# reidprichard/ORC

Hardware: AMD Instinct MI355X
Metric: SIMPLE iterations/s (10.24M-cell hex channel equivalents; = iterations/s at N=1) (higher is better)
Workload: dtype f64

## Files before the change

orc_amd/csrc/linalg_kernels.hpp:

```cpp
#pragma once
#include "linalg.hpp"

namespace orc {

__device__ __forceinline__ double view_value(const MatView &A, int64_t row, int64_t pos) {
    double v = A.val[pos];
    if (A.s1) v = A.s1[row] * v;
    if (A.s2) v = A.s2[row] * v;
    return v;
}

template <bool NT, class T>
__device__ __forceinline__ T ld_stream(const T *p) {
    if (NT) return __builtin_nontemporal_load(p);
    return *p;
}

typedef unsigned u32x4_t __attribute__((ext_vector_type(4)));
typedef int i32x2_t __attribute__((ext_vector_type(2)));
typedef double f64x2_t __attribute__((ext_vector_type(2)));
typedef unsigned u32x3_t __attribute__((ext_vector_type(3)));
typedef u32x3_t u32x3_a4_t __attribute__((aligned(4)));
template <bool NT>
__device__ __forceinline__ u32x3_t ld_pos12(const unsigned *p) {
    if (NT) return __builtin_nontemporal_load(reinterpret_cast<const u32x3_a4_t *>(p));
    return *reinterpret_cast<const u32x3_a4_t *>(p);
}

__device__ __forceinline__ int packed_pair(bool in, int &off) {
    const unsigned long long m = __ballot(in);
    const int rank = __builtin_amdgcn_mbcnt_hi((unsigned)(m >> 32), __builtin_amdgcn_mbcnt_lo((unsigned)m, 0u));
    const int p = in ? off + rank : (m != 0ull ? off : off - 1);
    off += __popcll(m);
    return p;
}

__device__ __forceinline__ double fold_partials_block(const double *__restrict__ partials, int count, double *lds16 ) {
    const int lane = threadIdx.x & 63, w = threadIdx.x >> 6;
    double a[4], b[4];
#pragma unroll
    for (int p = 0; p < 4; ++p) {
        const int vt = (w + 4 * p) * 64 + lane;
        a[p] = vt < count ? partials[vt] : 0.;
        b[p] = vt + 1024 < count ? partials[vt + 1024] : 0.;
    }
    __syncthreads();
#pragma unroll
    for (int p = 0; p < 4; ++p) {
        const int vt = (w + 4 * p) * 64 + lane;
        double v = 0.;
        if (vt < count) v += a[p];
        if (vt + 1024 < count) v += b[p];
        v = wave_sum(v);
        if (lane == 0) lds16[w + 4 * p] = v;
    }
    __syncthreads();
    double r = 0.;
#pragma unroll
    for (int i = 0; i < 16; ++i) r += lds16[i];
    return r;
}

template <int NQ>
__device__ __forceinline__ void fold_partials_multi(const double *__restrict__ partials, int count, double *lds , double (&out)[NQ]) {
    const int lane = threadIdx.x & 63, w = threadIdx.x >> 6;
    double a[NQ][4], b[NQ][4];
#pragma unroll
    for (int q = 0; q < NQ; ++q) {
#pragma unroll
        for (int p = 0; p < 4; ++p) {
            const int vt = (w + 4 * p) * 64 + lane;
            a[q][p] = vt < count ? partials[(size_t)q * count + vt] : 0.;
            b[q][p] = vt + 1024 < count ? partials[(size_t)q * count + vt + 1024] : 0.;
        }
    }
    __syncthreads();
#pragma unroll
    for (int q = 0; q < NQ; ++q) {
#pragma unroll
        for (int p = 0; p < 4; ++p) {
            const int vt = (w + 4 * p) * 64 + lane;
            double v = 0.;
            if (vt < count) v += a[q][p];
            if (vt + 1024 < count) v += b[q][p];
            v = wave_sum(v);
            if (lane == 0) lds[q * 16 + w + 4 * p] = v;
        }
    }
    __syncthreads();
#pragma unroll
    for (int q = 0; q < NQ; ++q) {
        double r = 0.;
#pragma unroll
        for (int i = 0; i < 16; ++i) r += lds[q * 16 + i];
        out[q] = r;
    }
}

struct SliceWalk {
    int64_t begin, end, step;
    __device__ __forceinline__ SliceWalk(int32_t n_slices, int32_t first = 0) : SliceWalk(n_slices, first, (int)blockIdx.x, (int)gridDim.x) {}
    __device__ __forceinline__ SliceWalk(int32_t n_slices, int32_t first, int block, int grid) {
        const int waves = blockDim.x >> 6;
        const int wave = __builtin_amdgcn_readfirstlane((int)(threadIdx.x >> 6));
        if ((grid & 7) == 0 && grid >= 8) {
            const int xcd = block & 7, bl = block >> 3, nb = grid >> 3;
            const int64_t spx = ((int64_t)(n_slices - first) + 7) / 8;
            const int64_t lo = (int64_t)first + (int64_t)xcd * spx;
            int64_t hi = lo + spx;
            if (hi > n_slices) hi = n_slices;
            begin = lo + (int64_t)bl * waves + wave;
            end = hi;
            step = (int64_t)nb * waves;
        } else {
            begin = (int64_t)first + (int64_t)block * waves + wave;
            end = n_slices;
            step = (int64_t)grid * waves;
        }
    }
};

enum { kSpmvPlain = 0, kSpmvRagged = 1, kSpmvPacked = 2 };
template <class Epi, int kLayout = kSpmvPlain, bool kNoGather = false, bool kGuard = false>
__global__ __launch_bounds__(kBlock) void spmv_k(MatView A, const double *__restrict__ x, Epi epi, double *__restrict__ partials,
                                                 const double *__restrict__ skip_flags ) {
    __shared__ double lds[8];
    if (skip_flags && (skip_flags[0] != 0. || skip_flags[1] != 0.)) return;
    const int lane = threadIdx.x & 63;
    double r0 = 0., r1 = 0.;
    SliceWalk w(A.P.n_slices);
    for (int64_t slice = w.begin; slice < w.end; slice += w.step) {
        const int64_t row = slice * 64 + lane;
        const int64_t base = A.P.slice_ptr[slice];
        const int width = (int)((A.P.slice_ptr[slice + 1] - base) >> 6);
        const bool live = row < A.P.n;
        const int len = live ? A.P.row_len[row] : 0;
        const double s1 = (A.s1 && live) ? A.s1[row] : 1.;
        const double s2 = (A.s2 && live) ? A.s2[row] : 1.;
        double acc = 0.;
        const i32x2_t *pk_c = kLayout == kSpmvPacked ? reinterpret_cast<const i32x2_t *>(A.pk.col + A.pk.ptr[slice]) : nullptr;
        const f64x2_t *pk_v = kLayout == kSpmvPacked ? reinterpret_cast<const f64x2_t *>(A.pk.val + A.pk.ptr[slice]) : nullptr;
        int pk_off = 0;
        const int last = (kLayout == kSpmvRagged ? (len > 0 ? len : 1) : width) - 1;
        const int lane_c = live ? lane : (int)((A.P.n - 1) & 63);
        for (int k0 = 0; k0 < width; k0 += 8) {
            int c[8];
            double v[8], xv[8];
            if (kLayout == kSpmvPacked) {
#pragma unroll
                for (int q = 0; q < 4; ++q) {
                    const int p = packed_pair(k0 + 2 * q < len, pk_off);
                    const i32x2_t cc = pk_c[p];
                    const f64x2_t vv = pk_v[p];
                    c[2 * q] = cc.x; c[2 * q + 1] = cc.y;
                    v[2 * q] = vv.x; v[2 * q + 1] = vv.y;
                }
            } else {
#pragma unroll
                for (int u = 0; u < 8; ++u) {
                    if (kGuard) {
                        if (k0 + u < width) {
                            const int kk = kLayout == kSpmvPlain ? k0 + u : (k0 + u < last ? k0 + u : last);
                            const int64_t p = kLayout == kSpmvPlain ? (base + (int64_t)k0 * 64 + lane_c) + (int64_t)u * 64 : base + (int64_t)kk * 64 + lane_c;
                            c[u] = A.P.col[p];
                            v[u] = A.val[p];
                        } else { c[u] = 0; v[u] = 0.; }
                    } else {
                        const int kk = k0 + u < last ? k0 + u : last;
                        const int64_t p = base + (int64_t)kk * 64 + lane_c;
                        c[u] = A.P.col[p];
                        v[u] = A.val[p];
                    }
                }
            }
#pragma unroll
            for (int u = 0; u < 8; ++u) {
                if (kGuard) { if (k0 + u < width) xv[u] = x[c[u]]; else xv[u] = 0.; }
                else xv[u] = x[kNoGather ? (int)(live ? row : 0) + (c[u] & 0) : c[u]];
            }
#pragma unroll
            for (int u = 0; u < 8; ++u) {
                double t = v[u];
                if (A.s1) t = s1 * t;
                if (A.s2) t = s2 * t;
                const double next = acc + t * xv[u];
                acc = (k0 + u < len) ? next : acc;
            }
        }
        if (live) epi.apply(row, acc, r0, r1);
    }
    if (Epi::kReductions > 0) {
        double t = block_sum(r0, lds);
        if (threadIdx.x == 0) partials[blockIdx.x] = t;
    }
    if (Epi::kReductions > 1) {
        double t = block_sum(r1, lds);
        if (threadIdx.x == 0) partials[gridDim.x + blockIdx.x] = t;
    }
}

template <class Epi, bool kRagged = false, bool kMesh = false, bool kNarrow = false, bool kScaled = true, bool kNT = false>
__global__ __launch_bounds__(kBlock) void spmv_uniform_k(MatView A, const double *__restrict__ x, Epi epi, double *__restrict__ partials,
                                                 const double *__restrict__ skip_flags ) {
    __shared__ double lds[8];
    if (skip_flags && (skip_flags[0] != 0. || skip_flags[1] != 0.)) return;
    const int lane = threadIdx.x & 63;
    double r0 = 0., r1 = 0.;
    SliceWalk w(A.slice_hi >= 0 ? A.slice_hi : A.P.n_slices, A.slice_lo);
    for (int64_t slice = w.begin; slice < w.end; slice += w.step) {
        const int64_t row = slice * 64 + lane;
        const int64_t base = A.P.slice_ptr[slice];
        const int width = (int)((A.P.slice_ptr[slice + 1] - base) >> 6);
        const bool live = row < A.P.n;
        const int len = live ? A.P.row_len[row] : 0;
        const double s1 = (kScaled && A.s1 && live) ? A.s1[row] : 1.;
        const double s2 = (kScaled && A.s2 && live) ? A.s2[row] : 1.;
        double acc = 0.;
        const int32_t *__restrict__ cb = kNarrow ? A.P.colbase + (base >> 6) : nullptr;
        for (int k0 = 0; k0 < width; k0 += 8) {
            int c[8];
            double v[8], xv[8];
            const int64_t p0 = base + (int64_t)k0 * 64 + lane;
            if (kNarrow) {
#pragma unroll
                for (int u = 0; u < 8; ++u) {
                    const bool in = k0 + u < width;
                    c[u] = in ? cb[k0 + u] + (int)ld_stream<kNT>(A.P.col16 + p0 + (int64_t)u * 64) : 0;
                    v[u] = in ? ld_stream<kNT>(A.val + p0 + (int64_t)u * 64) : 0.;
                }
            } else {
#pragma unroll
                for (int u = 0; u < 8; ++u) {
                    const bool in = k0 + u < (kRagged ? len : width);
                    c[u] = in ? ld_stream<kNT>(A.P.col + p0 + (int64_t)u * 64) : 0;
                    v[u] = in ? ld_stream<kNT>(A.val + p0 + (int64_t)u * 64) : 0.;
                }
            }
#pragma unroll
            for (int u = 0; u < 8; ++u) xv[u] = (k0 + u < len) ? x[c[u]] : 0.;
#pragma unroll
            for (int u = 0; u < 8; ++u) {
                if (k0 + u < len) {
                    double t = v[u];
                    if (kScaled && A.s1) t = s1 * t;
                    if (kScaled && A.s2) t = s2 * t;
                    acc += t * xv[u];
                }
            }
        }
        if (live) epi.apply(row, acc, r0, r1);
    }
    const int pstride = A.part_stride > 0 ? A.part_stride : (int)gridDim.x;
    if (Epi::kReductions > 0) {
        double t = block_sum(r0, lds);
        if (threadIdx.x == 0) partials[A.part_base + blockIdx.x] = t;
    }
    if (Epi::kReductions > 1) {
        double t = block_sum(r1, lds);
        if (threadIdx.x == 0) partials[pstride + A.part_base + blockIdx.x] = t;
    }
}


struct __attribute__((aligned(8))) Vec3d { double a, b, c; };

template <class Epi3, int kChunk = 4, bool kMesh = false, bool kNarrow = false, bool kScaled = true, bool kNT = false>
__global__ __launch_bounds__(kBlock) void spmv3_uniform_k(MatView3 A, const double *__restrict__ x3, Epi3 epi, double *__restrict__ partials) {
    __shared__ double lds[8];
    const int lane = threadIdx.x & 63;
    const Vec3d *__restrict__ xv3 = reinterpret_cast<const Vec3d *>(x3);
    const Vec3d *__restrict__ s1v = reinterpret_cast<const Vec3d *>(A.s1);
    const Vec3d *__restrict__ s2v = reinterpret_cast<const Vec3d *>(A.s2);
    const int vgrid = (int)gridDim.x;
    for (int vb = blockIdx.x; vb < vgrid; vb += gridDim.x) {
    double red[3][2] = {{0., 0.}, {0., 0.}, {0., 0.}};
    SliceWalk w(A.slice_hi >= 0 ? A.slice_hi : A.P.n_slices, A.slice_lo, vb, vgrid);
    for (int64_t slice = w.begin; slice < w.end; slice += w.step) {
        const int64_t row = slice * 64 + lane;
        const int64_t base = A.P.slice_ptr[slice];
        const int width = (int)((A.P.slice_ptr[slice + 1] - base) >> 6);
        const bool live = row < A.P.n;
        const int len = live ? A.P.row_len[row] : 0;
        Vec3d s1 = {1., 1., 1.}, s2 = {1., 1., 1.};
        if (kScaled && A.s1 && live) s1 = s1v[row];
        if (kScaled && A.s2 && live) s2 = s2v[row];
        double acc0 = 0., acc1 = 0., acc2 = 0.;
        const int32_t *__restrict__ cb = kNarrow ? A.P.colbase + (base >> 6) : nullptr;
        for (int k0 = 0; k0 < width; k0 += kChunk) {
            int c[kChunk];
            double v0[kChunk], v1[kChunk], v2[kChunk];
            Vec3d xv[kChunk];
            const int64_t p0 = base + (int64_t)k0 * 64 + lane;
#pragma unroll
            for (int u = 0; u < kChunk; ++u) {
                const bool in = k0 + u < width;
                if (kNarrow) c[u] = in ? cb[k0 + u] + (int)ld_stream<kNT>(A.P.col16 + p0 + (int64_t)u * 64) : 0;
                else c[u] = in ? ld_stream<kNT>(A.P.col + p0 + (int64_t)u * 64) : 0;
                v0[u] = in ? ld_stream<kNT>(A.val[0] + p0 + (int64_t)u * 64) : 0.;
                v1[u] = in ? ld_stream<kNT>(A.val[1] + p0 + (int64_t)u * 64) : 0.;
                v2[u] = in ? ld_stream<kNT>(A.val[2] + p0 + (int64_t)u * 64) : 0.;
            }
#pragma unroll
            for (int u = 0; u < kChunk; ++u) {
                if (k0 + u < len) xv[u] = xv3[c[u]];
                else xv[u] = Vec3d{0., 0., 0.};
            }
#pragma unroll
            for (int u = 0; u < kChunk; ++u) {
                if (k0 + u < len) {
                    double t0 = v0[u], t1 = v1[u], t2 = v2[u];
                    if (kScaled && A.s1) { t0 = s1.a * t0; t1 = s1.b * t1; t2 = s1.c * t2; }
                    if (kScaled && A.s2) { t0 = s2.a * t0; t1 = s2.b * t1; t2 = s2.c * t2; }
                    acc0 += t0 * xv[u].a;
                    acc1 += t1 * xv[u].b;
                    acc2 += t2 * xv[u].c;
                }
            }
        }
        if (live) {
            const double acc[3] = {acc0, acc1, acc2};
            epi.apply(row, acc, red);
        }
    }
#pragma unroll
    for (int s = 0; s < 3; ++s) {
#pragma unroll
        for (int q = 0; q < Epi3::kReductions; ++q) {
            const double t = block_sum(red[s][q], lds);
            if (threadIdx.x == 0) partials[(size_t)(s * Epi3::kReductions + q) * (A.part_stride > 0 ? A.part_stride : vgrid) + A.part_base + vb] = t;
        }
    }
    }
}

template <class Epi, bool kScaled = true, bool kNT = false, bool kP12 = false>
__global__ __launch_bounds__(kBlock) void spmv_xwin_k(MatView A, const double *__restrict__ x, Epi epi, double *__restrict__ partials,
                                                      const double *__restrict__ skip_flags) {
    __shared__ double lds[8];
    extern __shared__ __align__(16) double xs[];
    constexpr int kC = kPackChunk;
    if (skip_flags && (skip_flags[0] != 0. || skip_flags[1] != 0.)) return;
    const int lane = threadIdx.x & 63, wave = __builtin_amdgcn_readfirstlane((int)(threadIdx.x >> 6));
    double r0 = 0., r1 = 0.;
    const int64_t n_blocks = ((int64_t)A.P.n_slices + 3) >> 2;
    int64_t b_begin, b_end, b_step;
    if ((gridDim.x & 7) == 0 && gridDim.x >= 8) {
        const int xcd = blockIdx.x & 7, bl = blockIdx.x >> 3, nb = gridDim.x >> 3;
        const int64_t per = (n_blocks + 7) / 8;
        b_begin = (int64_t)xcd * per + bl;
        b_end = (int64_t)(xcd + 1) * per < n_blocks ? (int64_t)(xcd + 1) * per : n_blocks;
        b_step = nb;
    } else {
        b_begin = blockIdx.x; b_end = n_blocks; b_step = gridDim.x;
    }
    for (int64_t b = b_begin; b < b_end; b += b_step) {
        const int ws_built = A.xw.wsize[b];
        const int ws = ws_built <= A.xw.cap ? ws_built : -1;
        const int64_t slice = b * 4 + wave;
        const bool has_slice = slice < A.P.n_slices;
        const int64_t row = slice * 64 + lane;
        const bool live = has_slice && row < A.P.n;
        int width = 0, len = 0;
        int64_t pk_off = 0, lp_off = 0;
        if (has_slice) {
            const int64_t base = A.P.slice_ptr[slice];
            width = (int)((A.P.slice_ptr[slice + 1] - base) >> 6);
            len = live ? A.P.row_len[row] : 0;
            pk_off = A.pk.ptr[slice];
            lp_off = ws >= 0 ? A.xw.lptr[slice] : 0;
        }
        const int64_t sb = __builtin_amdgcn_readfirstlane((int)(pk_off & 0xffffffff)) | ((int64_t)__builtin_amdgcn_readfirstlane((int)(pk_off >> 32)) << 32);
        const int64_t lb = __builtin_amdgcn_readfirstlane((int)(lp_off & 0xffffffff)) | ((int64_t)__builtin_amdgcn_readfirstlane((int)(lp_off >> 32)) << 32);
        const u32x4_t *s_pos = reinterpret_cast<const u32x4_t *>(A.xw.lidx + lb);
        const unsigned *s_pos12 = reinterpret_cast<const unsigned *>(A.xw.lidx) + (lb >> 3) * 3;
        const f64x2_t *s_val = reinterpret_cast<const f64x2_t *>(A.pk.val + sb);
        int poff = 0, voff = 0;
        u32x4_t c, cn;
        f64x2_t v[kC / 2], vn[kC / 2];
        auto issue = [&](int k0, u32x4_t &cc, f64x2_t (&vv)[kC / 2]) {
            {
                const unsigned long long m = __ballot(k0 < len);
                const int rank = __builtin_amdgcn_mbcnt_hi((unsigned)(m >> 32), __builtin_amdgcn_mbcnt_lo((unsigned)m, 0u));
                const int slot = poff + (k0 < len ? rank : 0);
                if (kP12) {
                    const u32x3_t w = ld_pos12<kNT>(s_pos12 + 3 * slot);
                    cc = u32x4_t{w.x, w.y, w.z, 0u};
                } else {
                    cc = ld_stream<kNT>(s_pos + slot);
                }
                poff += __popcll(m);
            }
#pragma unroll
            for (int q = 0; q < kC / 2; ++q) vv[q] = ld_stream<kNT>(s_val + packed_pair(k0 + 2 * q < len, voff));
        };
        if (ws > 0 && A.xw.wfmt[b]) {
            const int nseg = (ws + kXWinSeg - 1) / kXWinSeg;
            const int32_t *wb = A.xw.wcol + b * kXWinCap;
            const uint16_t *w16 = reinterpret_cast<const uint16_t *>(wb + nseg);
            for (int j0 = 0; j0 < ws; j0 += 8 * kBlock) {
                int wj[8];
                double xw[8];
#pragma unroll
                for (int q = 0; q < 8; ++q) {
                    const int j = j0 + q * kBlock + (int)threadIdx.x;
                    const int seg = min((j0 + q * kBlock + wave * 64) / kXWinSeg, nseg - 1);
                    wj[q] = wb[seg] + (int)ld_stream<kNT>(w16 + (j < ws ? j : ws - 1));
                }
#pragma unroll
                for (int q = 0; q < 8; ++q) xw[q] = x[wj[q]];
#pragma unroll
                for (int q = 0; q < 8; ++q) {
                    const int j = j0 + q * kBlock + (int)threadIdx.x;
                    if (j < ws) xs[j] = xw[q];
                }
            }
        } else if (ws > 0) {
            const int32_t *wc = A.xw.wcol + b * kXWinCap;
            for (int j0 = 0; j0 < ws; j0 += 8 * kBlock) {
                int wj[8];
                double xw[8];
#pragma unroll
                for (int q = 0; q < 8; ++q) {
                    const int j = j0 + q * kBlock + (int)threadIdx.x;
                    wj[q] = ld_stream<kNT>(wc + (j < ws ? j : 0));
                }
#pragma unroll
                for (int q = 0; q < 8; ++q) xw[q] = x[wj[q]];
#pragma unroll
                for (int q = 0; q < 8; ++q) {
                    const int j = j0 + q * kBlock + (int)threadIdx.x;
                    if (j < ws) xs[j] = xw[q];
                }
            }
        }
        __syncthreads();
        if (has_slice) {
            const double s1 = (kScaled && A.s1 && live) ? A.s1[row] : 1.;
            const double s2 = (kScaled && A.s2 && live) ? A.s2[row] : 1.;
            double acc = 0.;
            if (ws >= 0) {
                auto consume = [&](int k0, const u32x4_t &cc, const f64x2_t (&vv)[kC / 2]) {
                    double xv[kC];
                    if (kP12) {
                        const unsigned w0 = cc[0], w1 = cc[1], w2 = cc[2];
                        const unsigned o[kC] = {w0 << 3, w0 >> 9, __builtin_amdgcn_alignbit(w1, w0, 21), w1 >> 1, w1 >> 13, __builtin_amdgcn_alignbit(w2, w1, 25), w2 >> 5, w2 >> 17};
#pragma unroll
                        for (int u = 0; u < kC; ++u) xv[u] = *reinterpret_cast<const double *>(reinterpret_cast<const char *>(xs) + (o[u] & 0x7ff8u));
                    } else {
#pragma unroll
                        for (int q = 0; q < kC / 2; ++q) {
                            const unsigned w = cc[q];
                            xv[2 * q] = xs[w & 0xffffu];
                            xv[2 * q + 1] = xs[w >> 16];
                        }
                    }
#pragma unroll
                    for (int u = 0; u < kC; ++u) {
                        double t = vv[u >> 1][u & 1];
                        if (kScaled && A.s1) t = s1 * t;
                        if (kScaled && A.s2) t = s2 * t;
                        const double next = acc + t * xv[u];
                        acc = (k0 + u < len) ? next : acc;
                    }
                };
                if (width > 0) issue(0, c, v);
                int k0 = 0;
                for (; k0 + kC < width; k0 += 2 * kC) {
                    issue(k0 + kC, cn, vn);
                    consume(k0, c, v);
                    if (k0 + 2 * kC < width) issue(k0 + 2 * kC, c, v);
                    consume(k0 + kC, cn, vn);
                }
                if (k0 < width) consume(k0, c, v);
            } else {
                const i32x2_t *s_col = reinterpret_cast<const i32x2_t *>(A.pk.col + sb);
                for (int k0 = 0; k0 < width; k0 += 8) {
                    int cg[8];
                    double vg[8], xv[8];
#pragma unroll
                    for (int q = 0; q < 4; ++q) {
                        const int p = packed_pair(k0 + 2 * q < len, voff);
                        const i32x2_t cc = ld_stream<kNT>(s_col + p);
                        const f64x2_t vv = ld_stream<kNT>(s_val + p);
                        cg[2 * q] = cc.x; cg[2 * q + 1] = cc.y;
                        vg[2 * q] = vv.x; vg[2 * q + 1] = vv.y;
                    }
#pragma unroll
                    for (int u = 0; u < 8; ++u) xv[u] = x[cg[u]];
#pragma unroll
                    for (int u = 0; u < 8; ++u) {
                        double t = vg[u];
                        if (kScaled && A.s1) t = s1 * t;
                        if (kScaled && A.s2) t = s2 * t;
                        const double next = acc + t * xv[u];
                        acc = (k0 + u < len) ? next : acc;
                    }
                }
            }
            if (live) epi.apply(row, acc, r0, r1);
        }
        __syncthreads();
    }
    if (Epi::kReductions > 0 && A.xw.fold_scratch) {
        __shared__ int s_last;
        const int nwg = (int)gridDim.x;
        const double t0 = block_sum(r0, lds);
        const double t1 = Epi::kReductions > 1 ? block_sum(r1, lds) : 0.;
        if (threadIdx.x == 0) {
            __hip_atomic_store(A.xw.fold_scratch + blockIdx.x, t0, __ATOMIC_RELAXED, __HIP_MEMORY_SCOPE_AGENT);
            if (Epi::kReductions > 1) __hip_atomic_store(A.xw.fold_scratch + nwg + blockIdx.x, t1, __ATOMIC_RELAXED, __HIP_MEMORY_SCOPE_AGENT);
            __builtin_amdgcn_s_waitcnt(0);
            s_last = __hip_atomic_fetch_add(A.xw.fold_counter, 1u, __ATOMIC_RELAXED, __HIP_MEMORY_SCOPE_AGENT) == (unsigned)(nwg - 1);
        }
        __syncthreads();
        if (s_last) {
            const double *fs = A.xw.fold_scratch;
#pragma unroll
            for (int q = 0; q < Epi::kReductions; ++q) {
                double v = 0.;
                for (int i0 = threadIdx.x; i0 < nwg; i0 += 8 * kBlock) {
                    double t[8];
#pragma unroll
                    for (int u = 0; u < 8; ++u) {
                        const int i = i0 + u * kBlock;
                        t[u] = i < nwg ? __hip_atomic_load(fs + (size_t)q * nwg + i, __ATOMIC_RELAXED, __HIP_MEMORY_SCOPE_AGENT) : 0.;
                    }
#pragma unroll
                    for (int u = 0; u < 8; ++u) v += t[u];
                }
                v = block_sum(v, lds);
                if (threadIdx.x == 0) partials[q] = v;
            }
            if (threadIdx.x == 0) __hip_atomic_store(A.xw.fold_counter, 0u, __ATOMIC_RELAXED, __HIP_MEMORY_SCOPE_AGENT);
        }
        return;
    }
    if (Epi::kReductions > 0) {
        double t = block_sum(r0, lds);
        if (threadIdx.x == 0) partials[blockIdx.x] = t;
    }
    if (Epi::kReductions > 1) {
        double t = block_sum(r1, lds);
        if (threadIdx.x == 0) partials[gridDim.x + blockIdx.x] = t;
    }
}

}
```

Baseline: 1.427.

## Rework 3-component SpMV inner loop with scalar loads, clamped indexing and LDS reductions

Rewrites the spmv3_uniform_k kernel. Slice pointers and column bases are now read through constant-address-space (scalar) loads. Per-element addresses use 32-bit offsets from per-slice base pointers, and the per-lane 'in' predicate is replaced by clamping the index to the last valid column. Masking moves from branches to selects on the accumulators, and out-of-range x gathers read a safe row. Per-thread reduction accumulators are moved into LDS, and the virtual-block loop is dropped. The aim is fewer VGPRs and SALU/VALU address computations, plus branchless gathers, at the cost of extra LDS traffic and redundant loads in padded slots.

```diff
diff --git a/orc_amd/csrc/linalg_kernels.hpp b/orc_amd/csrc/linalg_kernels.hpp
--- a/orc_amd/csrc/linalg_kernels.hpp
+++ b/orc_amd/csrc/linalg_kernels.hpp
@@ -14,6 +14,16 @@
 __device__ __forceinline__ T ld_stream(const T *p) {
     if (NT) return __builtin_nontemporal_load(p);
     return *p;
+}
+
+template <class T>
+__device__ __forceinline__ T ld_uniform(const T *p) {
+    return *(const __attribute__((address_space(4))) T *)p;
+}
+
+template <bool NT, class T>
+__device__ __forceinline__ T ld_stream_at(const T *sbase, unsigned elem) {
+    return ld_stream<NT>(reinterpret_cast<const T *>(reinterpret_cast<const char *>(sbase) + (size_t)(elem * (unsigned)sizeof(T))));
 }
 
 typedef unsigned u32x4_t __attribute__((ext_vector_type(4)));
@@ -266,70 +276,78 @@
 
 template <class Epi3, int kChunk = 4, bool kMesh = false, bool kNarrow = false, bool kScaled = true, bool kNT = false>
 __global__ __launch_bounds__(kBlock) void spmv3_uniform_k(MatView3 A, const double *__restrict__ x3, Epi3 epi, double *__restrict__ partials) {
+    constexpr int kRed = 3 * Epi3::kReductions, kPer = Epi3::kReductions > 0 ? Epi3::kReductions : 1;
     __shared__ double lds[8];
+    __shared__ double red_lds[kRed > 0 ? kRed : 1][kBlock];
     const int lane = threadIdx.x & 63;
     const Vec3d *__restrict__ xv3 = reinterpret_cast<const Vec3d *>(x3);
     const Vec3d *__restrict__ s1v = reinterpret_cast<const Vec3d *>(A.s1);
     const Vec3d *__restrict__ s2v = reinterpret_cast<const Vec3d *>(A.s2);
-    const int vgrid = (int)gridDim.x;
-    for (int vb = blockIdx.x; vb < vgrid; vb += gridDim.x) {
-    double red[3][2] = {{0., 0.}, {0., 0.}, {0., 0.}};
-    SliceWalk w(A.slice_hi >= 0 ? A.slice_hi : A.P.n_slices, A.slice_lo, vb, vgrid);
+#pragma unroll
+    for (int q = 0; q < kRed; ++q) red_lds[q][threadIdx.x] = 0.;
+    SliceWalk w(A.slice_hi >= 0 ? A.slice_hi : A.P.n_slices, A.slice_lo);
     for (int64_t slice = w.begin; slice < w.end; slice += w.step) {
         const int64_t row = slice * 64 + lane;
-        const int64_t base = A.P.slice_ptr[slice];
-        const int width = (int)((A.P.slice_ptr[slice + 1] - base) >> 6);
+        const int64_t base = ld_uniform(A.P.slice_ptr + slice);
+        const int width = (int)((ld_uniform(A.P.slice_ptr + slice + 1) - base) >> 6);
         const bool live = row < A.P.n;
         const int len = live ? A.P.row_len[row] : 0;
         Vec3d s1 = {1., 1., 1.}, s2 = {1., 1., 1.};
         if (kScaled && A.s1 && live) s1 = s1v[row];
         if (kScaled && A.s2 && live) s2 = s2v[row];
         double acc0 = 0., acc1 = 0., acc2 = 0.;
-        const int32_t *__restrict__ cb = kNarrow ? A.P.colbase + (base >> 6) : nullptr;
+        const double *__restrict__ sv0 = A.val[0] + base, *__restrict__ sv1 = A.val[1] + base, *__restrict__ sv2 = A.val[2] + base;
+        const uint16_t *__restrict__ sc16 = kNarrow ? A.P.col16 + base : nullptr;
+        const int32_t *cb = kNarrow ? A.P.colbase + (base >> 6) : nullptr;
+        const int32_t *__restrict__ sc32 = kNarrow ? nullptr : A.P.col + base;
+        const int safe = live ? (int)row : 0;
         for (int k0 = 0; k0 < width; k0 += kChunk) {
             int c[kChunk];
+            unsigned e[kChunk];
             double v0[kChunk], v1[kChunk], v2[kChunk];
             Vec3d xv[kChunk];
-            const int64_t p0 = base + (int64_t)k0 * 64 + lane;
+            const int last = width - 1 - k0;
 #pragma unroll
             for (int u = 0; u < kChunk; ++u) {
-                const bool in = k0 + u < width;
-                if (kNarrow) c[u] = in ? cb[k0 + u] + (int)ld_stream<kNT>(A.P.col16 + p0 + (int64_t)u * 64) : 0;
-                else c[u] = in ? ld_stream<kNT>(A.P.col + p0 + (int64_t)u * 64) : 0;
-                v0[u] = in ? ld_stream<kNT>(A.val[0] + p0 + (int64_t)u * 64) : 0.;
-                v1[u] = in ? ld_stream<kNT>(A.val[1] + p0 + (int64_t)u * 64) : 0.;
-                v2[u] = in ? ld_stream<kNT>(A.val[2] + p0 + (int64_t)u * 64) : 0.;
+                const int d = k0 + (u < last ? u : last);
+                e[u] = (unsigned)d * 64u + (unsigned)lane;
+                if (kNarrow) c[u] = ld_uniform(cb + d) + (int)ld_stream_at<kNT>(sc16, e[u]);
+                else c[u] = ld_stream_at<kNT>(sc32, e[u]);
             }
 #pragma unroll
             for (int u = 0; u < kChunk; ++u) {
-                if (k0 + u < len) xv[u] = xv3[c[u]];
-                else xv[u] = Vec3d{0., 0., 0.};
-            }
+                v0[u] = ld_stream_at<kNT>(sv0, e[u]);
+                v1[u] = ld_stream_at<kNT>(sv1, e[u]);
+                v2[u] = ld_stream_at<kNT>(sv2, e[u]);
+            }
+#pragma unroll
+            for (int u = 0; u < kChunk; ++u) xv[u] = xv3[k0 + u < len ? c[u] : safe];
 #pragma unroll
             for (int u = 0; u < kChunk; ++u) {
-                if (k0 + u < len) {
-                    double t0 = v0[u], t1 = v1[u], t2 = v2[u];
-                    if (kScaled && A.s1) { t0 = s1.a * t0; t1 = s1.b * t1; t2 = s1.c * t2; }
-                    if (kScaled && A.s2) { t0 = s2.a * t0; t1 = s2.b * t1; t2 = s2.c * t2; }
-                    acc0 += t0 * xv[u].a;
-                    acc1 += t1 * xv[u].b;
-                    acc2 += t2 * xv[u].c;
-                }
+                double t0 = v0[u], t1 = v1[u], t2 = v2[u];
+                if (kScaled && A.s1) { t0 = s1.a * t0; t1 = s1.b * t1; t2 = s1.c * t2; }
+                if (kScaled && A.s2) { t0 = s2.a * t0; t1 = s2.b * t1; t2 = s2.c * t2; }
+                const double n0 = acc0 + t0 * xv[u].a, n1 = acc1 + t1 * xv[u].b, n2 = acc2 + t2 * xv[u].c;
+                const bool in = k0 + u < len;
+                acc0 = in ? n0 : acc0;
+                acc1 = in ? n1 : acc1;
+                acc2 = in ? n2 : acc2;
             }
         }
         if (live) {
             const double acc[3] = {acc0, acc1, acc2};
+            double red[3][2] = {{0., 0.}, {0., 0.}, {0., 0.}};
+#pragma unroll
+            for (int q = 0; q < kRed; ++q) red[q / kPer][q % kPer] = red_lds[q][threadIdx.x];
             epi.apply(row, acc, red);
-        }
-    }
-#pragma unroll
-    for (int s = 0; s < 3; ++s) {
-#pragma unroll
-        for (int q = 0; q < Epi3::kReductions; ++q) {
-            const double t = block_sum(red[s][q], lds);
-            if (threadIdx.x == 0) partials[(size_t)(s * Epi3::kReductions + q) * (A.part_stride > 0 ? A.part_stride : vgrid) + A.part_base + vb] = t;
-        }
-    }
+#pragma unroll
+            for (int q = 0; q < kRed; ++q) red_lds[q][threadIdx.x] = red[q / kPer][q % kPer];
+        }
+    }
+#pragma unroll
+    for (int q = 0; q < kRed; ++q) {
+        const double t = block_sum(red_lds[q][threadIdx.x], lds);
+        if (threadIdx.x == 0) partials[(size_t)q * (A.part_stride > 0 ? A.part_stride : (int)gridDim.x) + A.part_base + blockIdx.x] = t;
     }
 }
 
```

Result: no change. 1.436, median of 6 (+0.7%).
